# zju3dv/neuralbody

Hardware: NVIDIA H100
Metric: rays_per_s_512x512_64spp (higher is better)
Workload: dtype f16x2 (hi+lo fp16 pairs, fp32 accumulate)

## Files before the change

neuralbody_b200/csrc/nb_capi.cu:

```cuda
#include <stdarg.h>
#include <stdio.h>
#include "nb_device.cuh"
#include "nb_train.h"

namespace nb {

static thread_local char g_err[512] = "";

void set_error(const char* fmt, ...) {
    va_list ap;
    va_start(ap, fmt);
    vsnprintf(g_err, sizeof(g_err), fmt, ap);
    va_end(ap);
}

template <typename OT>
__device__ __forceinline__ OT cvt_out(float v);
template <>
__device__ __forceinline__ float cvt_out<float>(float v) { return v; }
template <>
__device__ __forceinline__ __half cvt_out<__half>(float v) { return __float2half_rn(v); }

template <typename OT>
__global__ void __launch_bounds__(256) pack_volume_kernel(const float* __restrict__ src, OT* __restrict__ dst, int C,
// ... 184 lines not shown
    near[idx] = tn;
    far[idx] = tf;
    mask[idx] = hit ? 1 : 0;
}

__global__ void gen_rays_sharded_kernel(nb_camera cam, int rank, int world, int chunk, int n_local, float* __restrict__ ray_o,
                                        float* __restrict__ ray_d, float* __restrict__ near, float* __restrict__ far,
                                        unsigned char* __restrict__ mask) {
    const int j = blockIdx.x * blockDim.x + threadIdx.x;
    if (j >= n_local) return;
    const long long pix = ((long long)(j / chunk) * world + rank) * chunk + j % chunk;
    float of[3] = {0.f, 0.f, 0.f}, df[3] = {0.f, 0.f, 1.f}, tn = 0.f, tf = 0.f;
    bool hit = false;
    if (pix < (long long)cam.H * cam.W) {
        hit = gen_ray(cam, (int)pix, of, df, tn, tf);
        if (!hit) tn = tf = 0.f;
    }
    for (int a = 0; a < 3; ++a) { ray_o[j * 3 + a] = of[a]; ray_d[j * 3 + a] = df[a]; }
    near[j] = tn;
    far[j] = tf;
    mask[j] = hit ? 1 : 0;
}

__device__ __forceinline__ __half f16_hi(float x) { return __float2half_rn(x); }
__device__ __forceinline__ __half f16_lo(float x) { return __float2half_rn(x - __half2float(__float2half_rn(x))); }

__global__ void stream_kernel(nb_decoder_weights w, const float* __restrict__ f32, const float* __restrict__ bc,
                              __half* __restrict__ seq, __half* __restrict__ frame_steps) {
    const int stride = gridDim.x * blockDim.x;
    const int t0 = blockIdx.x * blockDim.x + threadIdx.x;
    for (int layer = 0; layer < 3; ++layer) {
        const int K = layer == 0 ? kFeat : kHidden;
        const int nks = K / 16;
        const float* W = layer == 0 ? w.fc0_w : layer == 1 ? w.fc1_w : w.fc2_w;
        const float* Bv = layer == 0 ? w.fc0_b : layer == 1 ? w.fc1_b : w.fc2_b;
        __half* dst = seq + (layer == 0 ? sL0 : layer == 1 ? sL1 : sL2);
        for (int i = t0; i < (2 * nks + 1) * 256 * 16; i += stride) {
            const int sl = i / 4096, n = (i / 16) % 256, kk = i % 16;
            const int half = n >> 7, nl = n & 127;
            if (sl < 2 * nks) {
                const int ks = sl >> 1, lo = sl & 1;
                const int k = ks * 16 + kk;
                const float x = W[(size_t)n * K + (layer == 0 ? feat_tc_to_orig(k) : k)];
                dst[pair_step_offset(ks, lo, half, nks) + step_offset(nl, kk, 128)] = lo ? f16_lo(x) : f16_hi(x);
            } else {
                dst[pair_bias_offset(half, nks) + step_offset(nl, kk, 128)] =
                    kk == 0 ? f16_hi(Bv[n]) : kk == 1 ? f16_lo(Bv[n]) : __float2half_rn(0.f);
            }
        }
    }
    for (int i = t0; i < (kStepsL3 - 1 + w.batch) * kN3 * 16; i += stride) {
        int st = i / (kN3 * 16);
        const int n = (i / 16) % kN3, kk = i % 16;
        const int half = n / (kN3 / 2), nl = n % (kN3 / 2);
        int b = 0;
        __half* dst;
        if (st >= kStepsL3 - 1) { b = st - (kStepsL3 - 1); st = kStepsL3 - 1; dst = frame_steps + ((size_t)b * 2 + half) * kHalfTile3; }
        else dst = seq + sL3 + pair_l3_offset(st, half);
        float v = 0.f;
        bool lo = false;
        if (st < 16) {
            v = f32[oWct + (size_t)(st * 16 + kk) * kColor + n];
        } else {
            const int k2 = (st - 16) * 16 + kk;
            if (k2 < kXyzPE) v = w.view_w[n * 346 + 283 + k2];
            else if (k2 >= 64 && k2 < 64 + kViewPE) v = w.view_w[n * 346 + 256 + (k2 - 64)];
            else if (k2 == 92) v = bc[b * kColor + n];
            else if (k2 == 93) { v = bc[b * kColor + n]; lo = true; }
        }
        dst[step_offset(nl, kk, kN3 / 2)] = lo ? f16_lo(v) : f16_hi(v);
    }
}

}

using namespace nb;

extern "C" {

int nb_abi_version(void) { return NB_ABI_VERSION; }
const char* nb_last_error(void) { return g_err; }
int nb_has_precision(int precision) {
    if (precision == NB_PRECISION_FP32) return 1;
    if (precision == NB_PRECISION_TC_FP16 || precision == NB_PRECISION_TC_FP16X3 || precision == NB_PRECISION_TC_TF32X3) return tc_available() ? 1 : 0;
    return 0;
}

static size_t dtype_size(int dtype) { return dtype == NB_DTYPE_F16 ? 2 : 4; }

size_t nb_packed_volume_level_offset(const int dims[NB_NUM_LEVELS][4], int batch, int dtype, int level) {
    size_t off = 0;
    for (int l = 0; l < level && l < NB_NUM_LEVELS; ++l)
        off += align256((size_t)batch * dims[l][0] * dims[l][1] * dims[l][2] * dims[l][3] * dtype_size(dtype));
    return off;
}

static size_t vox_words(const int d[4]) { return ((size_t)d[1] * d[2] * d[3] + 31) / 32; }
static size_t cell_words(const int d[4]) { return ((size_t)(d[1] + 1) * (d[2] + 1) * (d[3] + 1) + 31) / 32; }
static size_t occ_offset(const int dims[NB_NUM_LEVELS][4], int batch, int dtype, int level, int cell) {
    size_t off = nb_packed_volume_level_offset(dims, batch, dtype, NB_NUM_LEVELS);
    for (int l = 0; l < NB_NUM_LEVELS; ++l) {
        if (l == level && !cell) return off;
        off += align256((size_t)batch * vox_words(dims[l]) * 4);
        if (l == level && cell) return off;
        off += align256((size_t)batch * cell_words(dims[l]) * 4);
    }
    return off;
}

size_t nb_packed_volume_bytes(const int dims[NB_NUM_LEVELS][4], int batch, int dtype) {
    return occ_offset(dims, batch, dtype, NB_NUM_LEVELS, 0);
}

int nb_pack_volume(const nb_volume_level levels[NB_NUM_LEVELS], int batch, int dtype, void* out_blob, size_t out_bytes,
                   void* stream) {
    if (!levels || !out_blob || batch <= 0) { set_error("nb_pack_volume: null argument or batch <= 0"); return NB_ERR_BAD_ARG; }
    if (dtype != NB_DTYPE_F32 && dtype != NB_DTYPE_F16) { set_error("nb_pack_volume: unknown dtype %d", dtype); return NB_ERR_BAD_ARG; }
    int dims[NB_NUM_LEVELS][4];
    for (int l = 0; l < NB_NUM_LEVELS; ++l) {
        if (!levels[l].data || levels[l].C <= 0 || levels[l].C % 8 || levels[l].D <= 0 || levels[l].H <= 0 || levels[l].W <= 0) {
            set_error("nb_pack_volume: level %d has a null pointer or bad dims (C must be a multiple of 8)", l);
            return NB_ERR_BAD_ARG;
        }
// ... 218 lines not shown
```

neuralbody_b200/csrc/nb_layout.h:

```cpp
#pragma once
#include <stddef.h>

namespace nb {

constexpr int kFeat = 352;
constexpr int kHidden = 256;
constexpr int kColor = 128;
constexpr int kXyzPE = 63;
constexpr int kViewPE = 27;
constexpr int kColorK = 320;

constexpr int kSaveF = 0;
constexpr int kSaveH0 = kSaveF + kFeat;
constexpr int kSaveH1 = kSaveH0 + kHidden;
constexpr int kSaveH2 = kSaveH1 + kHidden;
constexpr int kSaveW = kSaveH2 + kColorK;
constexpr int kSaveDim = kSaveW + kColor;
constexpr int kGradRaw = 0, kGradW = 4, kGradH2 = kGradW + kColor, kGradH1 = kGradH2 + kHidden,
              kGradH0 = kGradH1 + kHidden, kGradDim = kGradH0 + kHidden;

constexpr size_t oW0t = 0;
constexpr size_t oB0 = oW0t + (size_t)kFeat * kHidden;
constexpr size_t oW1t = oB0 + kHidden;
constexpr size_t oB1 = oW1t + (size_t)kHidden * kHidden;
constexpr size_t oW2t = oB1 + kHidden;
constexpr size_t oB2 = oW2t + (size_t)kHidden * kHidden;
constexpr size_t oAlphaW = oB2 + kHidden;
constexpr size_t oAlphaB = oAlphaW + kHidden;
constexpr size_t oWct = oAlphaB + 4;
constexpr size_t oWvt = oWct + (size_t)kColorK * kColor;
constexpr size_t oRgbW = oWvt + (size_t)28 * kColor;
constexpr size_t oRgbB = oRgbW + 3 * kColor;
constexpr size_t oWc = oRgbB + 4;
constexpr size_t oSigmaEmpty = oWc + (size_t)kColor * kHidden;
constexpr size_t kF32Floats = oSigmaEmpty + 4;

__host__ __device__ inline long long clamp_latent(long long li, int num_train_frame) {
    return li < 0 ? 0 : li >= num_train_frame ? num_train_frame - 1 : li;
}

constexpr size_t kF16ByteOffset = ((kF32Floats * 4 + 255) / 256) * 256;
constexpr int kKsL0 = 22, kKsL12 = 16;
constexpr int kStepsL3 = 22, kStepsL4 = 9;
constexpr int kN3 = 128, kN4 = 16;
constexpr int kPeK = 96;
constexpr size_t kStepHalves256 = 256 * 16, kStepHalves3 = kN3 * 16, kStepHalves4 = kN4 * 16;
constexpr size_t sL0 = 0;
constexpr size_t sL1 = sL0 + (2 * kKsL0 + 1) * kStepHalves256;
constexpr size_t sL2 = sL1 + (2 * kKsL12 + 1) * kStepHalves256;
constexpr size_t sL3 = sL2 + (2 * kKsL12 + 1) * kStepHalves256;
constexpr size_t sL4 = sL3 + kStepsL3 * kStepHalves3;
constexpr size_t kF16Halves = sL4 + kStepsL4 * kStepHalves4;

__host__ __device__ inline int feat_tc_to_orig(int j) {
    return j < 128 ? 224 + j : j < 256 ? 96 + (j - 128) : j < 320 ? 32 + (j - 256) : j - 320;
}
__host__ __device__ inline int class_segments(int c) { return c == 0 ? 6 : c == 1 ? 5 : c == 2 ? 4 : 2; }
__host__ __device__ inline int class_ksteps(int c) { return c == 0 ? 22 : c == 1 ? 20 : c == 2 ? 16 : 8; }

constexpr int kHalfTile256 = 128 * 16;
constexpr int kHalfTile3 = (kN3 / 2) * 16;
constexpr int kHalfTile4 = (kN4 / 2) * 16;
__host__ __device__ inline size_t pair_group_offset(int g0, int half, int nks) {
    const int g = g0 >> 2;
    const int gs = (nks - 4 * g) < 4 ? (nks - 4 * g) : 4;
    return (size_t)8 * g * kStepHalves256 + (size_t)half * 2 * gs * kHalfTile256;
}
__host__ __device__ inline size_t pair_step_offset(int ks, int lo, int half, int nks) {
    const int g = ks >> 2;
    const int gs = (nks - 4 * g) < 4 ? (nks - 4 * g) : 4;
    return pair_group_offset(4 * g, half, nks) + (size_t)((lo ? gs : 0) + (ks & 3)) * kHalfTile256;
}
__host__ __device__ inline size_t pair_bias_offset(int half, int nks) { return (size_t)2 * nks * kStepHalves256 + (size_t)half * kHalfTile256; }
__host__ __device__ inline size_t pair_l3_offset(int step, int half) { return (size_t)half * (kStepsL3 - 1) * kHalfTile3 + (size_t)step * kHalfTile3; }
__host__ __device__ inline size_t pair_l4_offset(int step, int half) { return (size_t)half * kStepsL4 * kHalfTile4 + (size_t)step * kHalfTile4; }

__host__ __device__ inline size_t step256_offset(int ks, int lo, int nks) {
    const int g = ks >> 2;
    const int gsteps = (nks - 4 * g) < 4 ? (nks - 4 * g) : 4;
    return ((size_t)8 * g + (lo ? gsteps : 0) + (ks & 3)) * kStepHalves256;
}
__host__ __device__ inline size_t bias256_offset(int nks) { return (size_t)2 * nks * kStepHalves256; }

constexpr size_t kScratchByteOffset = ((kF16ByteOffset + kF16Halves * 2 + 255) / 256) * 256;
constexpr size_t kScratchDoubles = (size_t)kColor * kHidden;
constexpr size_t kBcByteOffset = kScratchByteOffset + kScratchDoubles * 8;

__host__ __device__ inline size_t u_byte_offset(int batch) {
    size_t b = kBcByteOffset + (size_t)batch * kColor * 4;
    return (b + 255) / 256 * 256;
}
__host__ __device__ inline size_t frame_step_byte_offset(int batch) {
    size_t b = u_byte_offset(batch) + (size_t)batch * kHidden * 8;
    return (b + 255) / 256 * 256;
}
__host__ __device__ inline size_t packed_weights_bytes(int batch) {
    return frame_step_byte_offset(batch) + (size_t)batch * kStepHalves3 * 2;
}

__host__ __device__ inline size_t step_offset(int n, int kk, int N) {
    return ((size_t)(kk >> 3) * (N >> 3) + (n >> 3)) * 64 + (size_t)(n & 7) * 8 + (kk & 7);
}

__host__ __device__ inline size_t umma_kmajor_offset(int n, int k, int N) {
    return ((size_t)(k >> 3) * (N >> 3) + (n >> 3)) * 64 + (size_t)(n & 7) * 8 + (k & 7);
}

}
```

neuralbody_b200/csrc/nb_render_tc_list.cu:

```cuda
#include "nb_tc_common.cuh"
#include <type_traits>

namespace nb {
namespace tcl {

using tcr::Quad;

constexpr int TP = 128;
constexpr int NUM_SEGS = 6;

__device__ __forceinline__ unsigned long long global_ns() {
    unsigned long long t;
    asm volatile("mov.u64 %0, %%globaltimer;" : "=l"(t));
    return t;
}

constexpr int CLS_THREADS = 256;

__device__ __forceinline__ uint32_t occupied_levels(const RenderParams& P, int b, float gx, float gy, float gz) {
    const uint32_t* occ_base = reinterpret_cast<const uint32_t*>(P.volume);
    uint32_t lm = 0;
#pragma unroll
    for (int lvl = 0; lvl < 4; ++lvl) {
        const int D = P.lvl_D[lvl], H = P.lvl_H[lvl], W = P.lvl_W[lvl];
// ... 71 lines not shown
            const float ox = __ldg(P.ray_o + ri * 3), oy = __ldg(P.ray_o + ri * 3 + 1), oz = __ldg(P.ray_o + ri * 3 + 2);
            const float dx = __ldg(P.ray_d + ri * 3), dy = __ldg(P.ray_d + ri * 3 + 1), dz = __ldg(P.ray_d + ri * 3 + 2);
            const float z = z_sample(__ldg(P.near + ri), __ldg(P.far + ri), P.t_vals, s, S, P.t_rand ? P.t_rand + ri * S : nullptr, P.z_user ? P.z_user + ri * S : nullptr);
            gm[k].x = __fadd_rn(ox, __fmul_rn(dx, z));
            gm[k].y = __fadd_rn(oy, __fmul_rn(dy, z));
            gm[k].z = __fadd_rn(oz, __fmul_rn(dz, z));
            float gx, gy, gz;
            world_to_grid(xf, gm[k].x, gm[k].y, gm[k].z, gx, gy, gz);
            const bool inside = P.mask_nv == 0 || inside_masks(P, xf, gm[k].x, gm[k].y, gm[k].z);
            const uint32_t lm = inside ? occupied_levels(P, b, gx, gy, gz) : 0u;
            if (inside && (lm != 0u || !can_skip)) cls[k] = (lm && !P.train_list) ? __ffs((int)lm) - 1 : 3;
            gm[k].w = __uint_as_float(((uint32_t)((r0 + ry) * S + s) + id0) | (lm << 28));
        }
    }
    append_to_lists(P, gm, cls);
    const float4 empty = make_float4(0.f, 0.f, 0.f, fminf(__ldg(P.wf32 + oSigmaEmpty), 0.f));
#pragma unroll
    for (int k = 0; k < CLS_PER_THREAD; ++k)
        if (cls[k] < 0 && live[k]) P.raw_ws[(__float_as_uint(gm[k].w) & kListIdMask) - id0] = empty;
}

__global__ void __launch_bounds__(CLS_THREADS) classify_points_kernel(const __grid_constant__ RenderParams P) {
    __shared__ FrameXf xf;
    const int tid = threadIdx.x;
    const int b = P.frame, n = P.n_points;
    const int i = blockIdx.x * CLS_THREADS + tid;
    load_frame_xf(P, b, xf, tid);
    __syncthreads();
    float4 e[1] = {make_float4(0.f, 0.f, 0.f, 0.f)};
    int cls[1] = {-1};
    if (i < n) {
        const float* q = P.points + (size_t)i * 3;
        e[0].x = __ldg(q); e[0].y = __ldg(q + 1); e[0].z = __ldg(q + 2);
        float gx, gy, gz;
        world_to_grid(xf, e[0].x, e[0].y, e[0].z, gx, gy, gz);
        const uint32_t lm = occupied_levels(P, b, gx, gy, gz);
        if (lm != 0u || !P.skip_empty) cls[0] = lm ? __ffs((int)lm) - 1 : 3;
        e[0].w = __uint_as_float((uint32_t)i | (lm << 28));
    }
    append_to_lists(P, e, cls);
    if (cls[0] < 0 && i < n) P.sigma[i] = __ldg(P.wf32 + oSigmaEmpty);
}

constexpr int NT = 384;
constexpr int NROWT = 96;
constexpr int LAUNCH_REGS = (65536 / NT) / 8 * 8;
constexpr int PRODUCER_REGS = 56, CONSUMER_REGS = 224;
constexpr int CHUNK_STRIDE = TP * 16 + 16;
constexpr int ACT_CHUNKS = kHidden / 8;
constexpr int PLANE_BYTES = ACT_CHUNKS * CHUNK_STRIDE;
constexpr int SEG_BUFS = 4;
constexpr int SLOT_BYTES = 16384, NUM_SLOTS = 4;
constexpr int TILE256 = kHalfTile256 * 2;
constexpr int TILE3 = kHalfTile3 * 2;
constexpr int L3_PUSH = 4;
constexpr int L3_PUSHES = (kStepsL3 + L3_PUSH - 1) / L3_PUSH;
constexpr int HEAD_FLOATS = kHidden + 4 + 3 * kColor + 4 + 3 * kHidden;
constexpr int H_ALPHA = 0, H_RGBW = kHidden + 4, H_RGBB = H_RGBW + 3 * kColor, H_B0 = H_RGBB + 4;
constexpr int OFF_HI = 0, OFF_LO = PLANE_BYTES;
constexpr int OFF_RING = 2 * PLANE_BYTES;
constexpr int OFF_HEAD = OFF_RING + NUM_SLOTS * SLOT_BYTES;
constexpr int OFF_XF = OFF_HEAD + HEAD_FLOATS * 4;
constexpr int OFF_SCHED = OFF_XF + 128;
constexpr int OFF_ROWS = OFF_SCHED + 64;
constexpr int NV_COARSE = 64, NV_FINE = 128;
__host__ __device__ constexpr int level_nv(int li) { return li < 2 ? NV_COARSE : NV_FINE; }
__host__ __device__ constexpr int level_channels(int li) { return li < 2 ? 128 : li == 2 ? 64 : 32; }
__host__ __device__ constexpr int ids_at(int li, int half) {
    return li < 2 ? (2 * li + half) * NV_COARSE : 4 * NV_COARSE + (2 * (li - 2) + half) * NV_FINE;
}
constexpr int HBITS = 8, HSIZE = 1 << HBITS;
constexpr uint32_t HEMPTY = 0xFFFFFFFFu;
struct VoxTable {
    float4 grid[TP];
    unsigned char slot[TP][4][8];
    uint32_t ids[ids_at(4, 0)];
    uint32_t n[8];
};
constexpr int OFF_VTAB = OFF_ROWS + 2 * TP * 16;
constexpr int OFF_HKEY = OFF_VTAB + 2 * (int)sizeof(VoxTable);
constexpr int OFF_HVAL = OFF_HKEY + 2 * HSIZE * 4;
constexpr int OFF_HCNT = OFF_HVAL + 2 * HSIZE;
constexpr int NCNT = 5;
constexpr int OFF_BAR = OFF_HCNT + 8 * 4;
enum { B_FULL = 0, B_EMPTY = B_FULL + NUM_SLOTS, B_ROWSFULL = B_EMPTY + NUM_SLOTS, B_L2DONE, B_PEFULL, B_ROWSFREE, NUM_BARS };
constexpr int SMEM_BYTES = OFF_BAR + NUM_BARS * 8;
static_assert(SMEM_BYTES <= 232448, "shared memory budget");
static_assert(OFF_RING % 128 == 0 && OFF_HEAD % 16 == 0 && OFF_ROWS % 16 == 0 && OFF_VTAB % 16 == 0 && OFF_HKEY % 16 == 0 &&
              OFF_BAR % 8 == 0, "alignment");
static_assert(NV_COARSE * level_channels(0) * 4 <= 2 * 2 * 8 * 1024 && NV_FINE * level_channels(2) * 4 <= 2 * 2 * 8 * 1024 &&
              NV_FINE < 255 && HSIZE > NV_FINE + 1 + NROWT && NCNT <= 8, "voxel staging");
static_assert(128 * PRODUCER_REGS + 256 * CONSUMER_REGS <= NT * LAUNCH_REGS, "register pool of the CTA");

__host__ __device__ constexpr int pushes_per_tile(int l0_ksteps) { return l0_ksteps + 2 * kKsL12 + L3_PUSHES; }

__device__ __forceinline__ uint32_t act_off(int row, int k) {
    return (uint32_t)((k >> 3) * CHUNK_STRIDE + (row >> 3) * 128 + (row & 7) * 16 + (k & 7) * 2);
}

__device__ __forceinline__ uint32_t clamped_cell(float gx, float gy, float gz, int W, int H, int D, Corners& cn) {
    corner_setup(unnormalize(gx, W), unnormalize(gy, H), unnormalize(gz, D), W, H, D, cn);
    auto axis = [](int i0, int size, float (&w)[2]) {
        if (i0 < 0) { w[0] = w[1]; w[1] = 0.f; return 0; }
        if (i0 >= size) { w[0] = w[1] = 0.f; return size - 2; }
        if (i0 == size - 1) { w[1] = w[0]; w[0] = 0.f; return size - 2; }
        return i0;
    };
    const int xc = axis(cn.x0, W, cn.wx), yc = axis(cn.y0, H, cn.wy), zc = axis(cn.z0, D, cn.wz);
    return (uint32_t)((zc * H + yc) * W + xc);
}

template <int NP, typename VT, bool DENSITY>
__device__ __forceinline__ void decode_list(const RenderParams& P) {
    extern __shared__ __align__(1024) unsigned char smem[];
    uint64_t* bars = reinterpret_cast<uint64_t*>(smem + OFF_BAR);
    FrameXf* xf = reinterpret_cast<FrameXf*>(smem + OFF_XF);
    float* head = reinterpret_cast<float*>(smem + OFF_HEAD);
    float4* rows_buf = reinterpret_cast<float4*>(smem + OFF_ROWS);
    const int tid = threadIdx.x, lane = tid & 31;
    const int warp = __shfl_sync(0xffffffffu, tid >> 5, 0);
    const int wgid = warp >> 2;
    const int S = P.n_samples;
    const uint32_t s_hi0 = tc::smem_u32(smem + OFF_HI), s_lo0 = tc::smem_u32(smem + OFF_LO), s_ring = tc::smem_u32(smem + OFF_RING);

    if (tid == 0) {
        for (int i = 0; i < NUM_SLOTS; ++i) {
            tc::mbar_init(&bars[B_FULL + i], 1);
            tc::mbar_init(&bars[B_EMPTY + i], 8);
        }
        tc::mbar_init(&bars[B_ROWSFULL], NROWT);
        tc::mbar_init(&bars[B_L2DONE], 8);
        tc::mbar_init(&bars[B_PEFULL], NROWT);
        tc::mbar_init(&bars[B_ROWSFREE], 8);
        tc::fence_mbar_init();
    }
    load_frame_xf(P, P.frame, *xf, tid);
    for (int i = tid; i < HEAD_FLOATS; i += NT) {
        float v;
        if (i < H_RGBW) v = __ldg(P.wf32 + oAlphaW + i);
        else if (i < H_B0) v = __ldg(P.wf32 + oRgbW + (i - H_RGBW));
        else {
            const int j = i - H_B0, l = j / kHidden, n = j % kHidden;
            v = __ldg(P.wf32 + (l == 0 ? oB0 : l == 1 ? oB1 : oB2) + n);
        }
        head[i] = v;
    }
    for (int i = tid; i < 2 * HSIZE; i += NT) reinterpret_cast<uint32_t*>(smem + OFF_HKEY)[i] = HEMPTY;
    if (tid < NCNT) reinterpret_cast<uint32_t*>(smem + OFF_HCNT)[tid] = 0u;
    struct Sched { unsigned int cnt[4]; int start[4]; int n_tiles; };
    Sched* sched = reinterpret_cast<Sched*>(smem + OFF_SCHED);
    if (tid == 0) {
        int acc = 0;
        for (int c = 0; c < 4; ++c) {
            const unsigned int n = P.list_count[c];
            sched->cnt[c] = n;
            sched->start[c] = acc;
            acc += (int)((n + TP - 1) / TP);
        }
        sched->n_tiles = acc;
        if (P.stats) atomicMax(P.frame_clock + 0, ~global_ns());
    }
    __syncthreads();
    const int n_tiles = sched->n_tiles;
    struct TileRef { int cls, nrows; const float4* ent; };
    auto tile_ref = [&](int tile) {
        TileRef r;
        r.cls = tile >= sched->start[3] ? 3 : tile >= sched->start[2] ? 2 : tile >= sched->start[1] ? 1 : 0;
        const int lt = tile - sched->start[r.cls];
        const unsigned int cnt = sched->cnt[r.cls];
        const long long rem = (long long)cnt - (long long)lt * TP;
        r.nrows = rem <= 0 ? 0 : rem < TP ? (int)rem : TP;
        const float4* buf = r.cls >= 2 ? P.list_a : P.list_b;
        r.ent = buf + ((r.cls & 1) ? (size_t)0 : P.list_cap - (size_t)cnt) + (size_t)lt * TP;
        return r;
    };

    if (wgid == 0) {
        tc::setmaxnreg_dec<PRODUCER_REGS>();
        const uint32_t s_hi = s_hi0, s_lo = s_lo0;
        if (warp == 0) {
            if (lane == 0) {
                tcr::Tracer tl;
                tl.init(P.trace, 3);
                const unsigned char* seq = reinterpret_cast<const unsigned char*>(P.wf16);
                unsigned long long real_tiles = 0, real_ksteps = 0;
                uint32_t g = 0;
                for (int tile = blockIdx.x; tile < n_tiles; tile += gridDim.x) {
                    const TileRef tref = tile_ref(tile);
                    const int l0_ksteps = class_ksteps(tref.cls);
                    real_tiles += tref.nrows > 0;
                    real_ksteps += tref.nrows > 0 ? l0_ksteps : 0;
                    const int npush = pushes_per_tile(l0_ksteps) - (DENSITY ? L3_PUSHES : 0);
                    for (int j = 0; j < npush; ++j, ++g) {
                        const uint32_t slot = g % NUM_SLOTS;
                        tc::mbar_wait(&bars[B_EMPTY + slot], ((g / NUM_SLOTS) & 1) ^ 1);
                        if (j == 0) tl.ev(1);
                        unsigned char* dst = smem + OFF_RING + slot * SLOT_BYTES;
                        uint64_t* bar = &bars[B_FULL + slot];
                        if (j < l0_ksteps + 2 * kKsL12) {
                            const int layer = j < l0_ksteps ? 0 : j < l0_ksteps + kKsL12 ? 1 : 2;
                            const int ks = layer == 0 ? j : layer == 1 ? j - l0_ksteps : j - l0_ksteps - kKsL12;
                            const int nks = layer == 0 ? kKsL0 : kKsL12;
                            const unsigned char* base = seq + 2 * (layer == 0 ? sL0 : layer == 1 ? sL1 : sL2);
                            tc::mbar_arrive_expect_tx(bar, (uint32_t)(2 * (NP == 3 ? 2 : 1) * TILE256));
#pragma unroll
                            for (int h = 0; h < 2; ++h)
#pragma unroll
                                for (int pl = 0; pl < (NP == 3 ? 2 : 1); ++pl)
                                    tc::bulk_g2s(dst + (2 * h + pl) * TILE256, base + 2 * pair_step_offset(ks, pl, h, nks), TILE256, bar);
                        } else {
                            const int g0 = (j - l0_ksteps - 2 * kKsL12) * L3_PUSH;
                            const int n = min(L3_PUSH, kStepsL3 - g0), common = min(n, kStepsL3 - 1 - g0);
                            const bool last = g0 + n == kStepsL3;
                            tc::mbar_arrive_expect_tx(bar, (uint32_t)(2 * n * TILE3));
#pragma unroll
                            for (int h = 0; h < 2; ++h) {
                                unsigned char* d = dst + h * (SLOT_BYTES / 2);
                                tc::bulk_g2s(d, seq + 2 * (sL3 + pair_l3_offset(g0, h)), common * TILE3, bar);
                                if (last)
                                    tc::bulk_g2s(d + common * TILE3, reinterpret_cast<const unsigned char*>(P.wframe) + ((size_t)P.frame * 2 + h) * TILE3,
                                                 TILE3, bar);
                            }
                        }
                    }
                    tl.ev(2);
                }
                if (P.stats) {
                    atomicAdd(P.stats + 0, real_tiles);
                    atomicAdd(P.stats + 4, real_ksteps);
                    if (blockIdx.x == 0) atomicAdd(P.stats + 1, (unsigned long long)sched->cnt[0] + sched->cnt[1] + sched->cnt[2] + sched->cnt[3]);
                }
            }
            __syncwarp();
        } else {
            const int pt = tid - 32;
            VoxTable* vtabs = reinterpret_cast<VoxTable*>(smem + OFF_VTAB);
            uint32_t* hkey = reinterpret_cast<uint32_t*>(smem + OFF_HKEY);
            unsigned char* hval = smem + OFF_HVAL;
            uint32_t* hcnt = reinterpret_cast<uint32_t*>(smem + OFF_HCNT);
            tcr::Tracer tr;
            tr.init(pt == 0 ? P.trace : nullptr, 0);
            auto pwait = [&](uint64_t* bar, uint32_t parity) { tc::mbar_wait_backoff(bar, parity, 64); };
            auto insert = [&](int half, uint32_t id, uint32_t* ids, uint32_t nv) -> uint32_t {
                if (*reinterpret_cast<volatile uint32_t*>(hcnt + half) > nv) return 0xFFu;
                uint32_t* keys = hkey + half * HSIZE;
                uint32_t h = (id * 2654435761u) >> (32 - HBITS);
#pragma unroll 1
                for (int p = 0; p < HSIZE; ++p, h = (h + 1) & (HSIZE - 1)) {
                    uint32_t k = *reinterpret_cast<volatile uint32_t*>(keys + h);
                    if (k == HEMPTY) k = atomicCAS(keys + h, HEMPTY, id);
                    if (k == HEMPTY) {
                        const uint32_t s = atomicAdd(hcnt + half, 1u);
                        if (s < nv) ids[s] = id;
                        hval[half * HSIZE + h] = (unsigned char)min(s, 255u);
                        return h;
                    }
                    if (k == id) return h;
                }
                return 0xFFu;
            };
            auto build_table = [&](VoxTable* vt, const float4* rows, int nrows, int nlev) {
                auto occupied = [&](int row, int lvl) { return row < nrows && ((__float_as_uint(rows[row].w) >> (28 + lvl)) & 1u); };
#pragma unroll 1
                for (int li = 0; li < nlev; ++li) {
                    const int lvl = 3 - li, D = P.lvl_D[lvl], H = P.lvl_H[lvl], W = P.lvl_W[lvl];
                    const uint32_t nv = (uint32_t)level_nv(li);
#pragma unroll 1
                    for (int j = pt; j < TP * 8; j += NROWT) {
                        const int row = j >> 3, c = j & 7;
                        uint32_t h = 0xFFu;
                        if (occupied(row, lvl)) {
                            const float4 gq = vt->grid[row];
                            Corners cn;
                            const uint32_t id = clamped_cell(gq.x, gq.y, gq.z, W, H, D, cn) + ((c & 1) ? 1u : 0u) +
                                                ((c & 2) ? (uint32_t)W : 0u) + ((c & 4) ? (uint32_t)(W * H) : 0u);
// ... 7 lines not shown
                        const int row = i >> 1;
                        uint32_t* wp = reinterpret_cast<uint32_t*>(&vt->slot[row][li][4 * (i & 1)]);
                        const unsigned char* hv = hval + (row >> 6) * HSIZE;
                        uint32_t out = 0xFFFFFFFFu;
                        if (occupied(row, lvl)) {
                            const uint32_t wd = *wp;
                            out = 0u;
#pragma unroll
                            for (int b = 0; b < 4; ++b) out |= (uint32_t)hv[(wd >> (8 * b)) & 0xFFu] << (8 * b);
                        }
                        *wp = out;
                    }
                    for (int i = pt; i < 2 * HSIZE; i += NROWT) hkey[i] = HEMPTY;
                    if (pt < 2) {
                        const uint32_t n = hcnt[pt];
                        vt->n[2 * li + pt] = n;
                        hcnt[pt] = 0u;
                        if (nrows > 64 * pt && (li < 2 || n > nv)) atomicAdd(hcnt + (li < 2 ? (n <= nv ? 2 : 3) : 4), 1u);
                    }
                    tcr::named_bar_sync(3, NROWT);
                }
            };
            auto load_rows = [&](int buf, int tile) {
                if (tile < n_tiles) {
                    const TileRef r = tile_ref(tile);
                    float4* dst = rows_buf + buf * TP;
                    VoxTable* vt = vtabs + buf;
                    for (int i = pt; i < TP; i += NROWT) {
                        const float4 e = i < r.nrows ? __ldg(r.ent + i) : make_float4(0.f, 0.f, 0.f, __uint_as_float(0xFFFFFFFFu));
                        dst[i] = e;
                        float gx, gy, gz;
                        world_to_grid(*xf, e.x, e.y, e.z, gx, gy, gz);
                        vt->grid[i] = make_float4(gx, gy, gz, 0.f);
                    }
                    tcr::named_bar_sync(3, NROWT);
                    build_table(vt, dst, r.nrows, 4 - r.cls);
                }
                tcr::named_bar_sync(3, NROWT);
                tc::mbar_arrive(&bars[B_ROWSFULL]);
            };

            int it = -1;
            for (int tile = (int)blockIdx.x - (int)gridDim.x; tile < n_tiles; tile += gridDim.x, ++it) {
                if (it >= 0) {
                    pwait(&bars[B_ROWSFREE], it & 1);
                    tr.ev(1);
                }
                load_rows((it + 1) & 1, tile + gridDim.x);
                if (DENSITY || it < 0) continue;
                tr.ev(30);
                const TileRef tref = tile_ref(tile);
                const int nrows = tref.nrows;
                const float4* rows = rows_buf + (it & 1) * TP;
                pwait(&bars[B_L2DONE], it & 1);
                tr.ev(31);
#pragma unroll 1
                for (int job = pt; job < 2 * TP; job += NROWT) {
                    const int prow = job % TP;
                    const float4 e = rows[prow];
                    auto put = [&](int k, float v) {
                        const __half hv = __float2half_rn(v);
                        asm volatile("st.shared.b16 [%0], %1;" ::"r"(s_lo + act_off(prow, k)), "h"(*reinterpret_cast<const unsigned short*>(&hv)) : "memory");
                    };
                    if (job < TP) {
                        positional_embed_anchored<10, 5>(e.x, e.y, e.z, [&](int j, float v) { put(j, v); });
                        put(63, 0.f);
                    } else {
                        const int smp = (int)(__float_as_uint(e.w) & kListIdMask);
                        const size_t ri = (size_t)P.frame * P.n_rays + (prow < nrows ? smp / S : 0);
                        const float dx = __ldg(P.ray_d + ri * 3), dy = __ldg(P.ray_d + ri * 3 + 1), dz = __ldg(P.ray_d + ri * 3 + 2);
                        const float nrm = ray_norm(dx, dy, dz);
                        positional_embed_anchored<4, 4>(__fdiv_rn(dx, nrm), __fdiv_rn(dy, nrm), __fdiv_rn(dz, nrm), [&](int j, float v) { put(64 + j, v); });
                        put(91, 0.f); put(92, 1.f); put(93, 1.f); put(94, 0.f); put(95, 0.f);
                    }
                }
                tc::fence_proxy_async();
                tc::mbar_arrive(&bars[B_PEFULL]);
                tr.ev(32);
            }
        }
    } else {
        tc::setmaxnreg_inc<CONSUMER_REGS>();
        uint32_t s_hi, s_lo;
        const int cw = wgid - 1;
        const bool arr = lane == 0;
        int tn = (!DENSITY && (tid & 127) == 0 && blockIdx.x == 0 && P.trace) ? (1 + cw) * 4096 : -1;
        auto tval = [&](int code, unsigned long long v) {
            if (tn >= 0 && tn < (2 + cw) * 4096) P.trace[tn++] = ((unsigned long long)code << 48) | (v & 0xFFFFFFFFFFFFull);
        };
        auto tev = [&](int code) { tval(code, (unsigned long long)clock64()); };
        const int r0 = 64 * cw + 16 * (warp & 3) + (lane >> 2), cq = 2 * (lane & 3);
        float acc0[64], acc1[64];
        auto init_bias = [&](const float* b) {
#pragma unroll
            for (int c = 0; c < 16; ++c) {
                const float2 v0 = *reinterpret_cast<const float2*>(b + 8 * c + cq), v1 = *reinterpret_cast<const float2*>(b + 128 + 8 * c + cq);
                acc0[4 * c] = v0.x; acc0[4 * c + 1] = v0.y; acc0[4 * c + 2] = v0.x; acc0[4 * c + 3] = v0.y;
                acc1[4 * c] = v1.x; acc1[4 * c + 1] = v1.y; acc1[4 * c + 2] = v1.x; acc1[4 * c + 3] = v1.y;
            }
        };
        const uint32_t wg_rows = (uint32_t)(cw * 8 * 128);
        auto mma256 = [&](uint32_t slot, int ka) {
            const uint64_t a_hi = tc::make_smem_desc(s_hi + wg_rows + 2 * ka * CHUNK_STRIDE, CHUNK_STRIDE, 128);
            const uint64_t a_lo = tc::make_smem_desc(s_lo + wg_rows + 2 * ka * CHUNK_STRIDE, CHUNK_STRIDE, 128);
            const uint64_t b0h = tc::make_smem_desc(slot + 0 * TILE256, 128 * 16, 128);
            const uint64_t b0l = tc::make_smem_desc(slot + 1 * TILE256, 128 * 16, 128);
// ... 150 lines not shown
                        }
#pragma unroll
                        for (int c = 0; c < 8; ++c) {
                            typename Quad<VT>::raw v0[2], v1[2];
#pragma unroll
                            for (int r = 0; r < 2; ++r) {
                                const uint32_t a = stage_addr((((c < 4) ? sl[r].x : sl[r].y) >> (8 * (c & 3))) & 0xFFu) + st_off;
                                v0[r] = Quad<VT>::load_shared(a);
                                v1[r] = nunits > 1 ? Quad<VT>::load_shared(a + 32 * sizeof(VT)) : Quad<VT>::zero();
                            }
#pragma unroll
                            for (int r = 0; r < 2; ++r)
                                if (cw8[r][c] != 0.f) {
                                    Quad<VT>::fma(acc[r][0], v0[r], cw8[r][c]);
                                    Quad<VT>::fma(acc[r][1], v1[r], cw8[r][c]);
                                }
                        }
                        store_row(row, acc[0]);
                        store_row(row + 16, acc[1]);
                    }
                } else {
                    const unsigned char* lvl_ptr = volbase + P.lvl_off[lvl] + ((size_t)P.frame * P.lvl_bstride[lvl] + 4 * t) * sizeof(VT);
                    const uint32_t dX = (uint32_t)(C * sizeof(VT)), dY = dX * W, dZ = dY * H;
                    for (int row = 64 * cw + grp; row < 64 * cw + 64; row += 16) {
                        const float4 e = rows[row];
                        const bool occ = row < nrows && ((__float_as_uint(e.w) >> (28 + lvl)) & 1u);
                        float acc[2][4] = {{0.f, 0.f, 0.f, 0.f}, {0.f, 0.f, 0.f, 0.f}};
                        if (occ) {
                            float gx, gy, gz;
                            world_to_grid(*xf, e.x, e.y, e.z, gx, gy, gz);
                            float cw8[8];
                            const uint32_t cb = setup(gx, gy, gz, cw8) * dX;
#pragma unroll
                            for (int uu = 0; uu < 2; ++uu) {
                                if (uu >= nunits) continue;
                                const unsigned char* ub = lvl_ptr + (size_t)(cbase0 + 32 * uu) * sizeof(VT);
                                typename Quad<VT>::raw v[8];
#pragma unroll
                                for (int c = 0; c < 8; ++c)
                                    v[c] = Quad<VT>::load_bytes(ub + cb + ((c & 1) ? dX : 0u) + ((c & 2) ? dY : 0u) + ((c & 4) ? dZ : 0u));
#pragma unroll
                                for (int c = 0; c < 8; ++c)
                                    if (cw8[c] != 0.f) Quad<VT>::fma(acc[uu], v[c], cw8[c]);
                            }
                        }
                        store_row(row, acc);
                    }
                }
            };

            {
                const uint32_t t0 = (uint32_t)clock();
                tc::mbar_wait(&bars[B_ROWSFULL], it & 1);
                r_stall += (uint32_t)clock() - t0;
            }
            __syncwarp();
            tc::mbar_arrive_if(&bars[B_ROWSFREE], arr);
            init_bias(head + H_B0);
            for (int seg = 0; seg < nseg; ++seg) {
                const uint32_t t0 = (uint32_t)clock();
                gather(seg);
                publish();
                (seg < 4 ? g_coarse : g_fine) += (uint32_t)clock() - t0;
                const int nks = seg == NUM_SEGS - 1 ? 2 : 4, ka = 4 * (seg % SEG_BUFS);
                for (int q = 0; q < nks; ++q) {
                    take([&](uint32_t slot) { mma256(slot, ka + q); });
                    tc::wgmma_wait<1>();
                    tc::acc_fence(acc0); tc::acc_fence(acc1);
                    release(g - 2, arr && q > 0);
                }
                tc::wgmma_wait<0>();
                tc::acc_fence(acc0); tc::acc_fence(acc1);
                release_last();
            }
            tev(20);
            convert(false);
            init_bias(head + H_B0 + kHidden);
            publish();
            float2 sig = make_float2(0.f, 0.f);
            for (int layer = 1; layer <= 2; ++layer) {
                for (int q = 0; q < kKsL12; ++q) {
                    take([&](uint32_t slot) { mma256(slot, q); });
                    tc::wgmma_wait<1>();
                    tc::acc_fence(acc0); tc::acc_fence(acc1);
                    release(g - 2, arr && q > 0);
                }
                tc::wgmma_wait<0>();
                tc::acc_fence(acc0); tc::acc_fence(acc1);
                release_last();
                tev(20 + layer);
                if (layer == 1) {
                    convert(false);
                    init_bias(head + H_B0 + 2 * kHidden);
                } else {
                    if (!DENSITY) tc::mbar_arrive_if(&bars[B_L2DONE], arr);
                    sig = convert(true);
                }
                publish();
            }
            if constexpr (DENSITY) {
                float sg[2] = {sig.x, sig.y};
#pragma unroll
                for (int hr = 0; hr < 2; ++hr) {
#pragma unroll
                    for (int o = 1; o <= 2; o <<= 1) sg[hr] += __shfl_xor_sync(0xffffffffu, sg[hr], o);
                    const int row = r0 + 8 * hr;
                    if ((lane & 3) == 0 && row < nrows) {
                        const uint32_t id = __float_as_uint(rows[row].w) & kListIdMask;
                        P.sigma[id] = sg[hr] + head[H_ALPHA + kHidden];
                    }
                }
                continue;
            }
            float c3a[32], c3b[32];
#pragma unroll
            for (int i = 0; i < 32; ++i) { c3a[i] = 0.f; c3b[i] = 0.f; }
#pragma unroll
            for (int p = 0; p < L3_PUSHES; ++p) {
                if (p * L3_PUSH == 16) {
                    const uint32_t t0 = (uint32_t)clock();
                    tc::mbar_wait(&bars[B_PEFULL], it & 1);
                    pe_stall += (uint32_t)clock() - t0;
                }
                take([&](uint32_t slot) {
#pragma unroll
                    for (int k = 0; k < L3_PUSH; ++k) {
                        const int ks = p * L3_PUSH + k;
                        if (ks >= kStepsL3) break;
                        const uint32_t a = ks < 16 ? s_hi + 2 * ks * CHUNK_STRIDE : s_lo + 2 * (ks - 16) * CHUNK_STRIDE;
                        const uint64_t ad = tc::make_smem_desc(a + wg_rows, CHUNK_STRIDE, 128);
                        tc::wgmma_m64n64k16_f16(c3a, ad, tc::make_smem_desc(slot + k * TILE3, 64 * 16, 128), true);
                        tc::wgmma_m64n64k16_f16(c3b, ad, tc::make_smem_desc(slot + SLOT_BYTES / 2 + k * TILE3, 64 * 16, 128), true);
                    }
                });
                tc::wgmma_wait<1>();
                tc::acc_fence(c3a); tc::acc_fence(c3b);
                release(g - 2, arr && p > 0);
            }
            tc::wgmma_wait<0>();
            tc::acc_fence(c3a); tc::acc_fence(c3b);
            release_last();
            tev(23);
            float cr[2] = {0.f, 0.f}, cg[2] = {0.f, 0.f}, cbl[2] = {0.f, 0.f};
            auto color = [&](const float (&a)[32], int nh) {
#pragma unroll
                for (int c = 0; c < 8; ++c) {
                    const int col = 64 * nh + 8 * c + cq;
                    const float2 w0 = *reinterpret_cast<const float2*>(head + H_RGBW + col);
                    const float2 w1 = *reinterpret_cast<const float2*>(head + H_RGBW + kColor + col);
                    const float2 w2 = *reinterpret_cast<const float2*>(head + H_RGBW + 2 * kColor + col);
#pragma unroll
                    for (int hr = 0; hr < 2; ++hr) {
                        const float x0 = fmaxf(a[4 * c + 2 * hr], 0.f), x1 = fmaxf(a[4 * c + 2 * hr + 1], 0.f);
                        cr[hr] = fmaf(x1, w0.y, fmaf(x0, w0.x, cr[hr]));
                        cg[hr] = fmaf(x1, w1.y, fmaf(x0, w1.x, cg[hr]));
                        cbl[hr] = fmaf(x1, w2.y, fmaf(x0, w2.x, cbl[hr]));
                    }
                }
            };
            color(c3a, 0);
            color(c3b, 1);
            float sg[2] = {sig.x, sig.y};
#pragma unroll
            for (int hr = 0; hr < 2; ++hr) {
#pragma unroll
                for (int o = 1; o <= 2; o <<= 1) {
                    cr[hr] += __shfl_xor_sync(0xffffffffu, cr[hr], o);
                    cg[hr] += __shfl_xor_sync(0xffffffffu, cg[hr], o);
                    cbl[hr] += __shfl_xor_sync(0xffffffffu, cbl[hr], o);
                    sg[hr] += __shfl_xor_sync(0xffffffffu, sg[hr], o);
                }
                const int row = r0 + 8 * hr;
                if ((lane & 3) == 0 && row < nrows) {
                    const int smp = (int)(__float_as_uint(rows[row].w) & kListIdMask);
                    P.raw_ws[smp] = make_float4(cr[hr] + head[H_RGBB], cg[hr] + head[H_RGBB + 1], cbl[hr] + head[H_RGBB + 2],
                                                sg[hr] + head[H_ALPHA + kHidden]);
                }
            }
            tev(24);
            tval(50, w_stall);
            tval(51, r_stall);
            tval(52, pe_stall);
            tval(53, g_coarse);
            tval(54, g_fine);
            w_stall = r_stall = pe_stall = g_coarse = g_fine = 0;
        }
    }
    __syncthreads();
    if (tid == 0 && P.stats) {
        atomicMax(P.frame_clock + 1, global_ns());
        const uint32_t* paths = reinterpret_cast<const uint32_t*>(smem + OFF_HCNT) + 2;
        atomicAdd(P.stats + 5, (unsigned long long)paths[0]);
        atomicAdd(P.stats + 6, (unsigned long long)paths[1]);
        atomicAdd(P.stats + 7, (unsigned long long)paths[2]);
    }
}

template <int NP, typename VT>
__global__ void __launch_bounds__(NT, 1) render_tc_list_kernel(const __grid_constant__ RenderParams P) {
    decode_list<NP, VT, false>(P);
}
template <int NP, typename VT>
__global__ void __launch_bounds__(NT, 1) density_tc_list_kernel(const __grid_constant__ RenderParams P) {
    decode_list<NP, VT, true>(P);
}

__device__ __forceinline__ void add_decoder_time(const RenderParams& P) {
    const unsigned long long t0 = ~P.frame_clock[0], t1 = P.frame_clock[1];
    atomicAdd(P.stats + 2, t1 > t0 ? t1 - t0 : 0ull);
    atomicAdd(P.stats + 3, 1ull);
}
__global__ void decoder_time_kernel(const __grid_constant__ RenderParams P) { add_decoder_time(P); }

constexpr int COMP_WARPS = 8;
__global__ void __launch_bounds__(COMP_WARPS * 32) composite_kernel(const __grid_constant__ RenderParams P) {
    __shared__ float zs[COMP_WARPS][kListMaxSamples];
    const int warp = threadIdx.x >> 5, lane = threadIdx.x & 31;
    const int ray = blockIdx.x * COMP_WARPS + warp;
    if (blockIdx.x == 0 && threadIdx.x == 0 && P.stats) add_decoder_time(P);
    if (ray >= P.n_rays) return;
    const int S = P.n_samples;
    const size_t rg = (size_t)P.frame * P.n_rays + ray;
    const float near = __ldg(P.near + rg), far = __ldg(P.far + rg);
    for (int s = lane; s < S; s += 32) zs[warp][s] = z_sample(near, far, P.t_vals, s, S, P.t_rand ? P.t_rand + rg * S : nullptr, P.z_user ? P.z_user + rg * S : nullptr);
    __syncwarp();
    const float dx = __ldg(P.ray_d + rg * 3), dy = __ldg(P.ray_d + rg * 3 + 1), dz = __ldg(P.ray_d + rg * 3 + 2);
    float* wout = P.weights ? P.weights + rg * S : nullptr;
    RayOut o = composite_ray(P.raw_ws + (size_t)ray * S, zs[warp], S, ray_norm(dx, dy, dz), wout, lane);
    if (lane == 0) store_ray_outputs(P, rg, o);
}

template <int NP, typename VT, bool DENSITY>
static cudaError_t launch_list(const RenderParams& p, int grid, cudaStream_t stream) {
    void (*kernel)(RenderParams) = DENSITY ? density_tc_list_kernel<NP, VT> : render_tc_list_kernel<NP, VT>;
    cudaError_t e = cudaFuncSetAttribute(kernel, cudaFuncAttributeMaxDynamicSharedMemorySize, SMEM_BYTES);
    if (e != cudaSuccess) return e;
    kernel<<<grid, NT, SMEM_BYTES, stream>>>(p);
// ... 119 lines not shown
```

Baseline: 16.00 million.

## Stream layer-3 per-point weight steps into lo plane instead of ring

The layer-3 color weights switch from a half-split layout to a contiguous per-step layout. Only the 16 h2 K-steps now go through the shared weight ring, and the remaining 6 per-point/view/frame steps are bulk-copied by the producer into spare chunks of the lo activation plane under new XFULL/XEMPTY barriers. This cuts the number of ring pushes and allows those loads to overlap the earlier layers. The change also adds L1 prefetches of ray directions in the PE warps. In exchange it brings in extra barrier synchronisation and reuses activation smem space, which could cause stalls.

```diff
diff --git a/neuralbody_b200/csrc/nb_capi.cu b/neuralbody_b200/csrc/nb_capi.cu
--- a/neuralbody_b200/csrc/nb_capi.cu
+++ b/neuralbody_b200/csrc/nb_capi.cu
@@ -260,11 +260,10 @@
     for (int i = t0; i < (kStepsL3 - 1 + w.batch) * kN3 * 16; i += stride) {
         int st = i / (kN3 * 16);
         const int n = (i / 16) % kN3, kk = i % 16;
-        const int half = n / (kN3 / 2), nl = n % (kN3 / 2);
         int b = 0;
         __half* dst;
-        if (st >= kStepsL3 - 1) { b = st - (kStepsL3 - 1); st = kStepsL3 - 1; dst = frame_steps + ((size_t)b * 2 + half) * kHalfTile3; }
-        else dst = seq + sL3 + pair_l3_offset(st, half);
+        if (st >= kStepsL3 - 1) { b = st - (kStepsL3 - 1); st = kStepsL3 - 1; dst = frame_steps + (size_t)b * kStepHalves3; }
+        else dst = seq + sL3 + l3_step_offset(st);
         float v = 0.f;
         bool lo = false;
         if (st < 16) {
@@ -276,7 +275,7 @@
             else if (k2 == 92) v = bc[b * kColor + n];
             else if (k2 == 93) { v = bc[b * kColor + n]; lo = true; }
         }
-        dst[step_offset(nl, kk, kN3 / 2)] = lo ? f16_lo(v) : f16_hi(v);
+        dst[step_offset(n, kk, kN3)] = lo ? f16_lo(v) : f16_hi(v);
     }
 }
 
diff --git a/neuralbody_b200/csrc/nb_layout.h b/neuralbody_b200/csrc/nb_layout.h
--- a/neuralbody_b200/csrc/nb_layout.h
+++ b/neuralbody_b200/csrc/nb_layout.h
@@ -59,7 +59,6 @@
 __host__ __device__ inline int class_ksteps(int c) { return c == 0 ? 22 : c == 1 ? 20 : c == 2 ? 16 : 8; }
 
 constexpr int kHalfTile256 = 128 * 16;
-constexpr int kHalfTile3 = (kN3 / 2) * 16;
 constexpr int kHalfTile4 = (kN4 / 2) * 16;
 __host__ __device__ inline size_t pair_group_offset(int g0, int half, int nks) {
     const int g = g0 >> 2;
@@ -72,7 +71,7 @@
     return pair_group_offset(4 * g, half, nks) + (size_t)((lo ? gs : 0) + (ks & 3)) * kHalfTile256;
 }
 __host__ __device__ inline size_t pair_bias_offset(int half, int nks) { return (size_t)2 * nks * kStepHalves256 + (size_t)half * kHalfTile256; }
-__host__ __device__ inline size_t pair_l3_offset(int step, int half) { return (size_t)half * (kStepsL3 - 1) * kHalfTile3 + (size_t)step * kHalfTile3; }
+__host__ __device__ inline size_t l3_step_offset(int step) { return (size_t)step * kStepHalves3; }
 __host__ __device__ inline size_t pair_l4_offset(int step, int half) { return (size_t)half * kStepsL4 * kHalfTile4 + (size_t)step * kHalfTile4; }
 
 __host__ __device__ inline size_t step256_offset(int ks, int lo, int nks) {
diff --git a/neuralbody_b200/csrc/nb_render_tc_list.cu b/neuralbody_b200/csrc/nb_render_tc_list.cu
--- a/neuralbody_b200/csrc/nb_render_tc_list.cu
+++ b/neuralbody_b200/csrc/nb_render_tc_list.cu
@@ -147,9 +147,12 @@
 constexpr int SEG_BUFS = 4;
 constexpr int SLOT_BYTES = 16384, NUM_SLOTS = 4;
 constexpr int TILE256 = kHalfTile256 * 2;
-constexpr int TILE3 = kHalfTile3 * 2;
+constexpr int TILE3 = kStepHalves3 * 2;
 constexpr int L3_PUSH = 4;
-constexpr int L3_PUSHES = (kStepsL3 + L3_PUSH - 1) / L3_PUSH;
+constexpr int L3_RING_STEPS = kKsL12;
+constexpr int L3_PUSHES = L3_RING_STEPS / L3_PUSH;
+constexpr int X_CHUNK0 = kPeK / 8;
+constexpr int X_STEPS = kStepsL3 - L3_RING_STEPS;
 constexpr int HEAD_FLOATS = kHidden + 4 + 3 * kColor + 4 + 3 * kHidden;
 constexpr int H_ALPHA = 0, H_RGBW = kHidden + 4, H_RGBB = H_RGBW + 3 * kColor, H_B0 = H_RGBB + 4;
 constexpr int OFF_HI = 0, OFF_LO = PLANE_BYTES;
@@ -178,7 +181,8 @@
 constexpr int OFF_HCNT = OFF_HVAL + 2 * HSIZE;
 constexpr int NCNT = 5;
 constexpr int OFF_BAR = OFF_HCNT + 8 * 4;
-enum { B_FULL = 0, B_EMPTY = B_FULL + NUM_SLOTS, B_ROWSFULL = B_EMPTY + NUM_SLOTS, B_L2DONE, B_PEFULL, B_ROWSFREE, NUM_BARS };
+enum { B_FULL = 0, B_EMPTY = B_FULL + NUM_SLOTS, B_ROWSFULL = B_EMPTY + NUM_SLOTS, B_L2DONE, B_PEFULL, B_ROWSFREE, B_XFULL, B_XEMPTY,
+       NUM_BARS };
 constexpr int SMEM_BYTES = OFF_BAR + NUM_BARS * 8;
 static_assert(SMEM_BYTES <= 232448, "shared memory budget");
 static_assert(OFF_RING % 128 == 0 && OFF_HEAD % 16 == 0 && OFF_ROWS % 16 == 0 && OFF_VTAB % 16 == 0 && OFF_HKEY % 16 == 0 &&
@@ -186,6 +190,9 @@
 static_assert(NV_COARSE * level_channels(0) * 4 <= 2 * 2 * 8 * 1024 && NV_FINE * level_channels(2) * 4 <= 2 * 2 * 8 * 1024 &&
               NV_FINE < 255 && HSIZE > NV_FINE + 1 + NROWT && NCNT <= 8, "voxel staging");
 static_assert(128 * PRODUCER_REGS + 256 * CONSUMER_REGS <= NT * LAUNCH_REGS, "register pool of the CTA");
+static_assert(L3_PUSHES * L3_PUSH == L3_RING_STEPS && L3_PUSH * TILE3 <= SLOT_BYTES && X_CHUNK0 + 2 * X_STEPS <= ACT_CHUNKS &&
+              L3_RING_STEPS == kKsL12 && kPeK == 16 * X_STEPS, "layer-3 weights: the h2 K-steps through the ring, the per-point tile's "
+              "through the lo plane");
 
 __host__ __device__ constexpr int pushes_per_tile(int l0_ksteps) { return l0_ksteps + 2 * kKsL12 + L3_PUSHES; }
 
@@ -227,6 +234,10 @@
         tc::mbar_init(&bars[B_L2DONE], 8);
         tc::mbar_init(&bars[B_PEFULL], NROWT);
         tc::mbar_init(&bars[B_ROWSFREE], 8);
+        if (!DENSITY) {
+            tc::mbar_init(&bars[B_XFULL], 1);
+            tc::mbar_init(&bars[B_XEMPTY], 8);
+        }
         tc::fence_mbar_init();
     }
     load_frame_xf(P, P.frame, *xf, tid);
@@ -280,7 +291,8 @@
                 const unsigned char* seq = reinterpret_cast<const unsigned char*>(P.wf16);
                 unsigned long long real_tiles = 0, real_ksteps = 0;
                 uint32_t g = 0;
-                for (int tile = blockIdx.x; tile < n_tiles; tile += gridDim.x) {
+                int it = 0;
+                for (int tile = blockIdx.x; tile < n_tiles; tile += gridDim.x, ++it) {
                     const TileRef tref = tile_ref(tile);
                     const int l0_ksteps = class_ksteps(tref.cls);
                     real_tiles += tref.nrows > 0;
@@ -305,17 +317,20 @@
                                     tc::bulk_g2s(dst + (2 * h + pl) * TILE256, base + 2 * pair_step_offset(ks, pl, h, nks), TILE256, bar);
                         } else {
                             const int g0 = (j - l0_ksteps - 2 * kKsL12) * L3_PUSH;
-                            const int n = min(L3_PUSH, kStepsL3 - g0), common = min(n, kStepsL3 - 1 - g0);
-                            const bool last = g0 + n == kStepsL3;
-                            tc::mbar_arrive_expect_tx(bar, (uint32_t)(2 * n * TILE3));
-#pragma unroll
-                            for (int h = 0; h < 2; ++h) {
-                                unsigned char* d = dst + h * (SLOT_BYTES / 2);
-                                tc::bulk_g2s(d, seq + 2 * (sL3 + pair_l3_offset(g0, h)), common * TILE3, bar);
-                                if (last)
-                                    tc::bulk_g2s(d + common * TILE3, reinterpret_cast<const unsigned char*>(P.wframe) + ((size_t)P.frame * 2 + h) * TILE3,
-                                                 TILE3, bar);
-                            }
+                            tc::mbar_arrive_expect_tx(bar, (uint32_t)(L3_PUSH * TILE3));
+                            tc::bulk_g2s(dst, seq + 2 * (sL3 + l3_step_offset(g0)), L3_PUSH * TILE3, bar);
+                        }
+                    }
+                    if (!DENSITY) {
+                        tc::mbar_wait(&bars[B_L2DONE], it & 1);
+                        uint64_t* bar = &bars[B_XFULL];
+                        tc::mbar_arrive_expect_tx(bar, (uint32_t)(X_STEPS * TILE3));
+#pragma unroll 1
+                        for (int x = 0; x < 2 * X_STEPS; ++x) {
+                            const int ks = L3_RING_STEPS + x / 2;
+                            const unsigned char* src = ks < kStepsL3 - 1 ? seq + 2 * (sL3 + l3_step_offset(ks))
+                                                                         : reinterpret_cast<const unsigned char*>(P.wframe) + (size_t)P.frame * TILE3;
+                            tc::bulk_g2s(smem + OFF_LO + (X_CHUNK0 + x) * CHUNK_STRIDE, src + (x & 1) * (TILE3 / 2), TILE3 / 2, bar);
                         }
                     }
                     tl.ev(2);
@@ -429,6 +444,15 @@
                 const TileRef tref = tile_ref(tile);
                 const int nrows = tref.nrows;
                 const float4* rows = rows_buf + (it & 1) * TP;
+#pragma unroll 1
+                for (int job = pt; job < 2 * TP; job += NROWT) {
+                    const int prow = job % TP;
+                    if (job < TP) continue;
+                    const int smp = (int)(__float_as_uint(rows[prow].w) & kListIdMask);
+                    const float* d = P.ray_d + ((size_t)P.frame * P.n_rays + (prow < nrows ? smp / S : 0)) * 3;
+                    asm volatile("prefetch.global.L1 [%0];" ::"l"(d));
+                    asm volatile("prefetch.global.L1 [%0];" ::"l"(d + 2));
+                }
                 pwait(&bars[B_L2DONE], it & 1);
                 tr.ev(31);
 #pragma unroll 1
@@ -685,6 +709,7 @@
             {
                 const uint32_t t0 = (uint32_t)clock();
                 tc::mbar_wait(&bars[B_ROWSFULL], it & 1);
+                if (!DENSITY && it > 0) tc::mbar_wait(&bars[B_XEMPTY], (it - 1) & 1);
                 r_stall += (uint32_t)clock() - t0;
             }
             __syncwarp();
@@ -745,34 +770,43 @@
                 }
                 continue;
             }
+            const uint32_t w_stall02 = w_stall;
             float c3a[32], c3b[32];
 #pragma unroll
             for (int i = 0; i < 32; ++i) { c3a[i] = 0.f; c3b[i] = 0.f; }
+            auto mma3 = [&](uint32_t a, uint32_t b, uint32_t lbo) {
+                const uint64_t ad = tc::make_smem_desc(a + wg_rows, CHUNK_STRIDE, 128);
+                tc::wgmma_m64n64k16_f16(c3a, ad, tc::make_smem_desc(b, lbo, 128), true);
+                tc::wgmma_m64n64k16_f16(c3b, ad, tc::make_smem_desc(b + 64 * 16, lbo, 128), true);
+            };
 #pragma unroll
             for (int p = 0; p < L3_PUSHES; ++p) {
-                if (p * L3_PUSH == 16) {
-                    const uint32_t t0 = (uint32_t)clock();
-                    tc::mbar_wait(&bars[B_PEFULL], it & 1);
-                    pe_stall += (uint32_t)clock() - t0;
-                }
                 take([&](uint32_t slot) {
 #pragma unroll
-                    for (int k = 0; k < L3_PUSH; ++k) {
-                        const int ks = p * L3_PUSH + k;
-                        if (ks >= kStepsL3) break;
-                        const uint32_t a = ks < 16 ? s_hi + 2 * ks * CHUNK_STRIDE : s_lo + 2 * (ks - 16) * CHUNK_STRIDE;
-                        const uint64_t ad = tc::make_smem_desc(a + wg_rows, CHUNK_STRIDE, 128);
-                        tc::wgmma_m64n64k16_f16(c3a, ad, tc::make_smem_desc(slot + k * TILE3, 64 * 16, 128), true);
-                        tc::wgmma_m64n64k16_f16(c3b, ad, tc::make_smem_desc(slot + SLOT_BYTES / 2 + k * TILE3, 64 * 16, 128), true);
-                    }
+                    for (int k = 0; k < L3_PUSH; ++k) mma3(s_hi + 2 * (p * L3_PUSH + k) * CHUNK_STRIDE, slot + k * TILE3, TILE3 / 2);
                 });
                 tc::wgmma_wait<1>();
                 tc::acc_fence(c3a); tc::acc_fence(c3b);
                 release(g - 2, arr && p > 0);
             }
+            {
+                const uint32_t t0 = (uint32_t)clock();
+                tc::mbar_wait(&bars[B_PEFULL], it & 1);
+                const uint32_t t1 = (uint32_t)clock();
+                pe_stall += t1 - t0;
+                tc::mbar_wait(&bars[B_XFULL], it & 1);
+                w_stall += (uint32_t)clock() - t1;
+            }
+            tc::wgmma_fence();
+#pragma unroll
+            for (int x = 0; x < X_STEPS; ++x) mma3(s_lo + 2 * x * CHUNK_STRIDE, s_lo + (X_CHUNK0 + 2 * x) * CHUNK_STRIDE, CHUNK_STRIDE);
+            tc::wgmma_commit();
+            tc::wgmma_wait<1>();
+            tc::acc_fence(c3a); tc::acc_fence(c3b);
+            release_last();
             tc::wgmma_wait<0>();
             tc::acc_fence(c3a); tc::acc_fence(c3b);
-            release_last();
+            tc::mbar_arrive_if(&bars[B_XEMPTY], arr);
             tev(23);
             float cr[2] = {0.f, 0.f}, cg[2] = {0.f, 0.f}, cbl[2] = {0.f, 0.f};
             auto color = [&](const float (&a)[32], int nh) {
@@ -811,11 +845,12 @@
                 }
             }
             tev(24);
-            tval(50, w_stall);
+            tval(50, w_stall02);
             tval(51, r_stall);
             tval(52, pe_stall);
             tval(53, g_coarse);
             tval(54, g_fine);
+            tval(55, w_stall - w_stall02);
             w_stall = r_stall = pe_stall = g_coarse = g_fine = 0;
         }
     }
```

Result: no change. 15.86 million, median of 6 (-0.9%).
